# lijrjyan/SDVAR

Measured on AMD Instinct MI355X. Metric: images/s (+ mean accepted tokens/step), VAR-d16 256^2 B=8, d12 draft + d16 verify, per GPU, higher is better.
Workload: dtype f32 (GEMM operands split into 2 fp16 planes to 2^-22, 3 fp16 MFMA products, fp32 accumulate); 1 GPU; BASELINE.json P1: VAR-d16 256^2 B=8/GPU, d12 draft + d16 verify, gamma=2, cfg=1.5 top_k=900 top_p=0.96, acceptance=natural, incl. VQVAE decode (overlapped with the next batch on a 2nd stream); verifier one round behind the draft once gamma = 1; parallelism=1 independent batch shards

## Files before the change

### sdvar_amd/csrc/conv.hip

```cpp
#include <stdlib.h>

#include "common.h"
#include "gemm_plan.h"

#ifdef SDVAR_TIMING_EXPERIMENTS
#define SDVAR_CDBG(a, bit) ((a).dbg & (bit))
#else
#define SDVAR_CDBG(a, bit) 0
#endif

namespace sdvar {


typedef __bf16 bf16x8 __attribute__((ext_vector_type(8)));
typedef _Float16 f16x8 __attribute__((ext_vector_type(8)));
typedef __attribute__((address_space(3))) void* lds_ptr_t;
typedef const __attribute__((address_space(1))) void* glb_ptr_t;

enum { CEPI_BIAS = 0, CEPI_BIAS_RES = 1, CEPI_PARTIAL = 2 };
constexpr int CBM = 256, CBN = 160;
constexpr int CSTAGE = 3 * (CBM + CBN) * 32;
constexpr int CSTAGE_H = 2 * (CBM + CBN) * 32;

struct ConvArgs {
    const uint16_t* X; const uint16_t* W;
    size_t xps, wps;
    size_t x_rows;
    int x_row0;
    const float* wsi;
    const float* bias; const float* res; float* out;
    int M, N, cb, taps, ih, iw, ldo, split, k_per_split;
    double* gn_part; int cpg;
    int up_phase;
    size_t w_phase_stride;
    int dbg;
};

__device__ __forceinline__ void conv_gn_store(const ConvArgs& a, const float* red, const float* piv, int n0, int tm, int phase, int tid) {
    const int col0 = tid * a.cpg;
    if (col0 < CBN && n0 + col0 < a.N) {
        const double n = 256.0, in = 1.0 / 256.0;
        double s = 0.0, m = 0.0;
        for (int c = col0; c < col0 + a.cpg; ++c) {
            double s1 = 0.0, s2 = 0.0;
            for (int w = 0; w < 8; ++w) { s1 += (double)red[w * 160 + c]; s2 += (double)red[1280 + w * 160 + c]; }
            const double sc = n * (double)piv[c] + s1;
            s += sc; m += s2 + (sc * sc - s1 * s1) * in;
        }
        double* o = a.gn_part + ((size_t)(a.up_phase >= 0 ? 4 * tm + phase : tm) * 32 + (n0 + col0) / a.cpg) * 2;
        o[0] = s; o[1] = m - s * s / (n * a.cpg);
    }
}

template <int EPI>
__device__ __forceinline__ void conv_epilogue(const ConvArgs& a, f32x16 (&acc)[5], float wsi, int m0, int n0, int tm, int ks, int phase, int wave, int li, int lh,
                                              int tid, uint16_t* csm) {
    float rv[5][16];
    if (EPI == CEPI_BIAS_RES) {
#pragma unroll
        for (int j = 0; j < 5; ++j) {
            const int n = n0 + j * 32 + li;
#pragma unroll
            for (int r = 0; r < 16; ++r) {
                const int m = m0 + wave * 32 + (r & 3) + 8 * (r >> 2) + 4 * lh;
                rv[j][r] = (n < a.N && m < a.M) ? a.res[(size_t)m * a.ldo + n] : 0.f;
            }
        }
    }
#pragma unroll
// ... 23 lines not shown
        if (wave == 0 && lh == 0) {
#pragma unroll
            for (int j = 0; j < 5; ++j) piv[j * 32 + li] = acc[j][0];
        }
        __syncthreads();
#pragma unroll
        for (int j = 0; j < 5; ++j) {
            float s1 = 0.f, s2 = 0.f;
            if (n0 + j * 32 + li < a.N) {
                const float K = piv[j * 32 + li];
#pragma unroll
                for (int r = 0; r < 16; ++r) { const float d = acc[j][r] - K; s1 += d; s2 += d * d; }
            }
            const auto w1 = __builtin_amdgcn_permlane32_swap(__float_as_uint(s1), __float_as_uint(s1), false, false);
            const auto w2 = __builtin_amdgcn_permlane32_swap(__float_as_uint(s2), __float_as_uint(s2), false, false);
            if (lh == 0) {
                red[wave * 160 + j * 32 + li] = __uint_as_float(w1[0]) + __uint_as_float(w1[1]);
                red[1280 + wave * 160 + j * 32 + li] = __uint_as_float(w2[0]) + __uint_as_float(w2[1]);
            }
        }
        __syncthreads();
        conv_gn_store(a, red, piv, n0, tm, phase, tid);
    }
}

typedef float cf32x4 __attribute__((ext_vector_type(4)));
__device__ __forceinline__ float dpp_row_sum16(float v) {
    v += __builtin_bit_cast(float, __builtin_amdgcn_update_dpp(0, __builtin_bit_cast(int, v), 0x111, 0xF, 0xF, true));
    v += __builtin_bit_cast(float, __builtin_amdgcn_update_dpp(0, __builtin_bit_cast(int, v), 0x112, 0xF, 0xF, true));
    v += __builtin_bit_cast(float, __builtin_amdgcn_update_dpp(0, __builtin_bit_cast(int, v), 0x114, 0xF, 0xF, true));
    v += __builtin_bit_cast(float, __builtin_amdgcn_update_dpp(0, __builtin_bit_cast(int, v), 0x118, 0xF, 0xF, true));
    return v;
}
template <int EPI>
__device__ __forceinline__ void conv_epilogue16(const ConvArgs& a, cf32x4 (&acc)[2][10], float wsi, int m0, int n0, int tm, int ks, int phase, int wave, int l15, int lq,
                                                int tid, uint16_t* csm) {
    int mrow[2]; size_t orow[2];
#pragma unroll
    for (int mt = 0; mt < 2; ++mt) {
        const int m = m0 + wave * 32 + 16 * mt + l15;
        mrow[mt] = m; orow[mt] = (size_t)m;
        if (EPI != CEPI_PARTIAL && a.up_phase >= 0 && m < a.M) {
            const int hw = a.ih * a.iw, b = m / hw, rem = m - b * hw, y = rem / a.iw, x = rem - y * a.iw;
            orow[mt] = ((size_t)(b * 2 * a.ih + 2 * y + (phase >> 1)) * (2 * a.iw) + 2 * x + (phase & 1));
        }
    }
    cf32x4 rv[2][10];
    if (EPI == CEPI_BIAS_RES) {
#pragma unroll
        for (int mt = 0; mt < 2; ++mt)
#pragma unroll
            for (int nt = 0; nt < 10; ++nt) {
                const int n = n0 + 16 * nt + 4 * lq;
                rv[mt][nt] = (n < a.N && mrow[mt] < a.M) ? *reinterpret_cast<const cf32x4*>(a.res + (size_t)mrow[mt] * a.ldo + n) : cf32x4{0.f, 0.f, 0.f, 0.f};
            }
    }
    float* outp = (EPI == CEPI_PARTIAL) ? a.out + (size_t)ks * a.M * a.ldo : a.out;
#pragma unroll
    for (int nt = 0; nt < 10; ++nt) {
        const int n = n0 + 16 * nt + 4 * lq;
        if (n >= a.N) continue;
        const cf32x4 bv = (EPI != CEPI_PARTIAL && a.bias) ? *reinterpret_cast<const cf32x4*>(a.bias + n) : cf32x4{0.f, 0.f, 0.f, 0.f};
#pragma unroll
        for (int mt = 0; mt < 2; ++mt) {
            if (mrow[mt] >= a.M) continue;
            cf32x4 v;
#pragma unroll
            for (int e = 0; e < 4; ++e) { v[e] = acc[mt][nt][e] * wsi + bv[e]; if (EPI == CEPI_BIAS_RES) v[e] += rv[mt][nt][e]; }
            if (!SDVAR_CDBG(a, 4)) *reinterpret_cast<cf32x4*>(outp + orow[mt] * a.ldo + n) = v;
            acc[mt][nt] = v;
        }
    }
    if (EPI != CEPI_PARTIAL && a.gn_part && !SDVAR_CDBG(a, 2)) {
        float* red = reinterpret_cast<float*>(csm);
        __shared__ __attribute__((aligned(16))) float piv[CBN];
        if (wave == 0 && l15 == 0) {
#pragma unroll
            for (int nt = 0; nt < 10; ++nt) *reinterpret_cast<cf32x4*>(piv + 16 * nt + 4 * lq) = acc[0][nt];
        }
        __syncthreads();
#pragma unroll
        for (int nt = 0; nt < 10; ++nt) {
            const bool in = n0 + 16 * nt + 4 * lq < a.N;
            const cf32x4 K = *reinterpret_cast<const cf32x4*>(piv + 16 * nt + 4 * lq);
#pragma unroll
            for (int e = 0; e < 4; ++e) {
                const float x0 = in ? acc[0][nt][e] - K[e] : 0.f, x1 = in ? acc[1][nt][e] - K[e] : 0.f;
                const float s1 = dpp_row_sum16(x0 + x1), s2 = dpp_row_sum16(x0 * x0 + x1 * x1);
                if (l15 == 15) { red[wave * 160 + 16 * nt + 4 * lq + e] = s1; red[1280 + wave * 160 + 16 * nt + 4 * lq + e] = s2; }
            }
        }
        __syncthreads();
        conv_gn_store(a, red, piv, n0, tm, phase, tid);
    }
}

template <int EPI>
__global__ __launch_bounds__(512, 2) void conv_bf16x3_kernel(ConvArgs a) {
    extern __shared__ __attribute__((aligned(16))) uint16_t csm[];
    const int tiles_m = (a.M + CBM - 1) / CBM, tiles_n = (a.N + CBN - 1) / CBN, ntile = tiles_m * tiles_n;
    const int ks = blockIdx.x / ntile;
    const int lid = xcd_remap(blockIdx.x - ks * ntile, ntile);
    const int tm = lid / tiles_n, tn = lid - tm * tiles_n;
// ... 88 lines not shown
                __builtin_amdgcn_sched_barrier(0);
                if (s == 0 && j == 0) {
                    SDVAR_LDS_RD(fb[1][1][4], ab1, 18432);
                    SDVAR_RD_B(1, ab1, 0, 0);
                }
                if (pf) {
                    const int grp = 5 * s + j;
                    issue_one(nst, grp);
                    if (grp >= 8) issue_one(nst, grp + 2);
                }
                __builtin_amdgcn_sched_barrier(0);
            }
        }
#undef SDVAR_RD_B
#undef SDVAR_LDS_RD
    }

    conv_epilogue<EPI>(a, acc, 1.0f, m0, n0, tm, ks, phase, wave, li, lh, tid, csm);
}

template <int EPI, int PP>
__global__ __launch_bounds__(512, 2) void conv_f16x2_kernel(ConvArgs a) {
    extern __shared__ __attribute__((aligned(16))) uint16_t csm[];
    const int tiles_m = (a.M + CBM - 1) / CBM, tiles_n = (a.N + CBN - 1) / CBN, ntile = tiles_m * tiles_n;
    const int ks = blockIdx.x / ntile;
    const int lid = xcd_remap(blockIdx.x - ks * ntile, ntile);
    const int tm = lid / tiles_n, tn = lid - tm * tiles_n;
    const int m0 = tm * CBM, n0 = tn * CBN;

    const int tid = threadIdx.x, lane = tid & 63, wave = tid >> 6;
    const int li = lane & 31, lh = lane >> 5;
    const int phase = a.up_phase >= 0 ? (int)blockIdx.y : 0;
    const uint16_t* Wp = a.W + (size_t)phase * a.w_phase_stride;

    const int r16 = lane >> 2;
    const int xr0 = 32 * wave + r16, xr1 = xr0 + 16, wr0 = 16 * wave + r16, wr1 = 128 + wr0;
    const int cx0 = (lane & 3) ^ ((xr0 >> 2) & 3), cx1 = (lane & 3) ^ ((xr1 >> 2) & 3), cw0 = (lane & 3) ^ ((wr0 >> 2) & 3), cw1 = (lane & 3) ^ ((wr1 >> 2) & 3);
    const int nkt = a.taps * a.cb;
    const int kt0 = ks * a.k_per_split;
    const int nk = min(nkt - kt0, a.k_per_split);
    const int w2 = a.iw + 2;
    auto prow = [&](int m) {
        const int hw = a.ih * a.iw, b = m / hw, rem = m - b * hw, y = rem / a.iw, x = rem - y * a.iw;
        return (size_t)(b * (a.ih + 2) + y + 1) * w2 + x + 1;
    };
    const int swave = __builtin_amdgcn_readfirstlane(wave);
    const uint32_t lx0 = (uint32_t)((a.x_row0 + prow(min(m0 + xr0, a.M - 1))) * 32 + 8 * cx0) * 2u;
    const uint32_t lx1 = (uint32_t)((a.x_row0 + prow(min(m0 + xr1, a.M - 1))) * 32 + 8 * cx1) * 2u;
    const uint32_t lw0 = (uint32_t)(min(n0 + wr0, a.N - 1) * 32 + 8 * cw0) * 2u, lw1 = (uint32_t)(min(n0 + wr1, a.N - 1) * 32 + 8 * cw1) * 2u;
    const bool two_w = swave < 2;
    const char* ux = nullptr; const char* uw = nullptr;
    const int tw = (a.taps == 9) ? 3 : 2;
    int sc = kt0 % a.cb, stap = kt0 / a.cb, sty = stap / tw, stx = stap - sty * tw, skb = kt0;
    auto set_next = [&]() {
        const int shift = (a.taps == 9) ? (sty - 1) * w2 + (stx - 1) : (a.taps == 4) ? (sty - 1 + (phase >> 1)) * w2 + (stx - 1 + (phase & 1)) : 0;
        ux = reinterpret_cast<const char*>(a.X) + ((long long)sc * (long long)a.x_rows + shift) * 64;
        uw = reinterpret_cast<const char*>(Wp) + (size_t)skb * a.N * 64;
        ++skb;
        if (++sc == a.cb) { sc = 0; if (++stx == tw) { stx = 0; ++sty; } }
    };
    auto issue_one = [&](uint16_t* st, int q) {
        if (q < 6) {
            const int p = q / 3, kind = q % 3;
            if (kind == 0) SDVAR_DMA16(lx0, ux + p * a.xps * 2, SDVAR_LDS_ADDR(st + p * 8192 + swave * 1024));
            else if (kind == 1) SDVAR_DMA16(lx1, ux + p * a.xps * 2, SDVAR_LDS_ADDR(st + p * 8192 + swave * 1024 + 512));
            else SDVAR_DMA16(lw0, uw + p * a.wps * 2, SDVAR_LDS_ADDR(st + 2 * 8192 + p * 5120 + swave * 512));
// ... 16 lines not shown
    set_next();
#pragma unroll
    for (int q = 0; q < 8; ++q) issue_one(csm, q);
    if (nk > 1) {
        set_next();
#pragma unroll
        for (int q = 0; q < 8; ++q) issue_one(csm + CSTAGE_H, q);
    }
    if constexpr (PP == 2) {
        const int late = __builtin_amdgcn_readfirstlane(wave >> 2);
        const int l15 = lane & 15, lq = lane >> 4;
        auto wait_next = [&](int t) {
            if (t + 2 < nk) { if (two_w) asm volatile("s_waitcnt vmcnt(8)" ::: "memory"); else asm volatile("s_waitcnt vmcnt(6)" ::: "memory"); }
            else asm volatile("s_waitcnt vmcnt(0)" ::: "memory");
        };
#define SDVAR_C_SLOT() do { __builtin_amdgcn_sched_barrier(0); __builtin_amdgcn_s_barrier(); __builtin_amdgcn_sched_barrier(0); } while (0)
#define SDVAR_LDS_RD(dst, addr, off) asm volatile("ds_read_b128 %0, %1 offset:" #off : "=v"(dst) : "v"(addr) : "memory")
#define SDVAR_C_MFMA16(J0)                                                                                      \
        _Pragma("unroll") for (int j = 0; j < 5; ++j)                                                           \
            _Pragma("unroll") for (int i = 0; i < 2; ++i) {                                                     \
                acc16[i][(J0) + j] = __builtin_amdgcn_mfma_f32_16x16x32_f16(fw[j][0], fx[i][1], acc16[i][(J0) + j], 0, 0, 0);   \
                acc16[i][(J0) + j] = __builtin_amdgcn_mfma_f32_16x16x32_f16(fw[j][1], fx[i][0], acc16[i][(J0) + j], 0, 0, 0);   \
                acc16[i][(J0) + j] = __builtin_amdgcn_mfma_f32_16x16x32_f16(fw[j][0], fx[i][0], acc16[i][(J0) + j], 0, 0, 0);   \
            }
        cf32x4 acc16[2][10];
#pragma unroll
        for (int i = 0; i < 2; ++i)
#pragma unroll
            for (int j = 0; j < 10; ++j)
#pragma unroll
                for (int r = 0; r < 4; ++r) acc16[i][j][r] = 0.f;
        const uint32_t fro = (uint32_t)(l15 * 64 + 16 * (lq ^ ((l15 >> 2) & 3)));
        const uint32_t fxo = (uint32_t)(wave * 32 * 64) + fro, fwo = 32768u + fro;
        wait_next(-1);
        SDVAR_C_SLOT();
        if (late) SDVAR_C_SLOT();
        f16x8 fx[2][2], fw[5][2];
#pragma unroll 1
        for (int t = 0; t < nk; ++t) {
            const bool pf = t + 2 < nk;
            uint16_t* nst = csm + ((t + 2) % 3) * CSTAGE_H;
            const uint32_t sb = (uint32_t)(uintptr_t)(lds_ptr_t)(csm + (t % 3) * CSTAGE_H);
            const uint32_t xa = sb + fxo, wa = sb + fwo;
            SDVAR_LDS_RD(fx[0][0], xa, 0); SDVAR_LDS_RD(fx[0][1], xa, 16384); SDVAR_LDS_RD(fx[1][0], xa, 1024); SDVAR_LDS_RD(fx[1][1], xa, 17408);
            SDVAR_LDS_RD(fw[0][0], wa, 0);    SDVAR_LDS_RD(fw[0][1], wa, 10240); SDVAR_LDS_RD(fw[1][0], wa, 1024); SDVAR_LDS_RD(fw[1][1], wa, 11264);
            SDVAR_LDS_RD(fw[2][0], wa, 2048); SDVAR_LDS_RD(fw[2][1], wa, 12288); SDVAR_LDS_RD(fw[3][0], wa, 3072); SDVAR_LDS_RD(fw[3][1], wa, 13312);
            SDVAR_LDS_RD(fw[4][0], wa, 4096); SDVAR_LDS_RD(fw[4][1], wa, 14336);
            if (pf) {
                set_next();
#pragma unroll
                for (int q = 0; q < 4; ++q) issue_one(nst, q);
            }
            asm volatile("s_waitcnt lgkmcnt(0)" ::: "memory");
            SDVAR_C_SLOT();
            SDVAR_C_MFMA16(0);
            SDVAR_C_SLOT();
            SDVAR_LDS_RD(fw[0][0], wa, 5120); SDVAR_LDS_RD(fw[0][1], wa, 15360); SDVAR_LDS_RD(fw[1][0], wa, 6144); SDVAR_LDS_RD(fw[1][1], wa, 16384);
            SDVAR_LDS_RD(fw[2][0], wa, 7168); SDVAR_LDS_RD(fw[2][1], wa, 17408); SDVAR_LDS_RD(fw[3][0], wa, 8192); SDVAR_LDS_RD(fw[3][1], wa, 18432);
            SDVAR_LDS_RD(fw[4][0], wa, 9216); SDVAR_LDS_RD(fw[4][1], wa, 19456);
            if (pf) {
#pragma unroll
                for (int q = 4; q < 8; ++q) issue_one(nst, q);
            }
            if (late) wait_next(t);
            asm volatile("s_waitcnt lgkmcnt(0)" ::: "memory");
            SDVAR_C_SLOT();
            SDVAR_C_MFMA16(5);
            if (!late) wait_next(t);
            SDVAR_C_SLOT();
        }
        if (!late) SDVAR_C_SLOT();
#undef SDVAR_C_MFMA16
#undef SDVAR_LDS_RD
#undef SDVAR_C_SLOT
        if (SDVAR_CDBG(a, 1)) return;
        conv_epilogue16<EPI>(a, acc16, a.wsi ? *a.wsi : 1.0f, m0, n0, tm, ks, phase, wave, l15, lq, tid, csm);
        return;
    } else
    if (PP) {
        const int late = __builtin_amdgcn_readfirstlane(wave >> 2);
        auto wait_next = [&](int t) {
            if (t + 2 < nk) { if (two_w) asm volatile("s_waitcnt vmcnt(8)" ::: "memory"); else asm volatile("s_waitcnt vmcnt(6)" ::: "memory"); }
            else asm volatile("s_waitcnt vmcnt(0)" ::: "memory");
        };
#define SDVAR_C_SLOT() do { __builtin_amdgcn_sched_barrier(0); __builtin_amdgcn_s_barrier(); __builtin_amdgcn_sched_barrier(0); } while (0)
#define SDVAR_LDS_RD(dst, addr, off) asm volatile("ds_read_b128 %0, %1 offset:" #off : "=v"(dst) : "v"(addr) : "memory")
#define SDVAR_RD_B(ab, p, pb) SDVAR_LDS_RD(fb[p][0], ab, pb); SDVAR_LDS_RD(fb[p][1], ab, pb + 2048); SDVAR_LDS_RD(fb[p][2], ab, pb + 4096); \
                              SDVAR_LDS_RD(fb[p][3], ab, pb + 6144); SDVAR_LDS_RD(fb[p][4], ab, pb + 8192)
#define SDVAR_C_MFMA()                                                                                  \
        _Pragma("unroll") for (int j = 0; j < 5; ++j) {                                                 \
            acc[j] = __builtin_amdgcn_mfma_f32_32x32x16_f16(fa[1], fb[0][j], acc[j], 0, 0, 0);          \
            acc[j] = __builtin_amdgcn_mfma_f32_32x32x16_f16(fa[0], fb[1][j], acc[j], 0, 0, 0);          \
            acc[j] = __builtin_amdgcn_mfma_f32_32x32x16_f16(fa[0], fb[0][j], acc[j], 0, 0, 0);          \
        }
        wait_next(-1);
        SDVAR_C_SLOT();
        if (late) SDVAR_C_SLOT();
        f16x8 fa[2], fb[2][5];
#pragma unroll 1
        for (int t = 0; t < nk; ++t) {
            const bool pf = t + 2 < nk;
            uint16_t* nst = csm + ((t + 2) % 3) * CSTAGE_H;
            const uint32_t sb = (uint32_t)(uintptr_t)(lds_ptr_t)(csm + (t % 3) * CSTAGE_H);
            const uint32_t aa0 = sb + 2 * (offa + ch0), aa1 = sb + 2 * (offa + ch1), ab0 = sb + 2 * (offb + ch0), ab1 = sb + 2 * (offb + ch1);
            SDVAR_LDS_RD(fa[0], aa0, 0); SDVAR_LDS_RD(fa[1], aa0, 16384);
            SDVAR_RD_B(ab0, 0, 0); SDVAR_RD_B(ab0, 1, 10240);
            if (pf) {
                set_next();
#pragma unroll
// ... 34 lines not shown
        f16x8 fa[2][2], fb[2][2][5];
#define SDVAR_LDS_RD(dst, addr, off) asm volatile("ds_read_b128 %0, %1 offset:" #off : "=v"(dst) : "v"(addr) : "memory")
#define SDVAR_RD_B(s, ab, p, pb) SDVAR_LDS_RD(fb[s][p][0], ab, pb); SDVAR_LDS_RD(fb[s][p][1], ab, pb + 2048); SDVAR_LDS_RD(fb[s][p][2], ab, pb + 4096); \
                                 SDVAR_LDS_RD(fb[s][p][3], ab, pb + 6144); SDVAR_LDS_RD(fb[s][p][4], ab, pb + 8192)
        SDVAR_LDS_RD(fa[0][0], aa0, 0); SDVAR_LDS_RD(fa[0][1], aa0, 16384);
        SDVAR_RD_B(0, ab0, 0, 0); SDVAR_RD_B(0, ab0, 1, 10240);
        SDVAR_LDS_RD(fa[1][0], aa1, 0); SDVAR_LDS_RD(fa[1][1], aa1, 16384);
        SDVAR_RD_B(1, ab1, 0, 0); SDVAR_RD_B(1, ab1, 1, 10240);
#undef SDVAR_RD_B
#undef SDVAR_LDS_RD
#pragma unroll
        for (int s = 0; s < 2; ++s) {
            if (s == 0) asm volatile("s_waitcnt lgkmcnt(12)" ::: "memory");
            else asm volatile("s_waitcnt lgkmcnt(0)" ::: "memory");
            __builtin_amdgcn_sched_barrier(0);
#pragma unroll
            for (int j = 0; j < 5; ++j) {
                acc[j] = __builtin_amdgcn_mfma_f32_32x32x16_f16(fa[s][1], fb[s][0][j], acc[j], 0, 0, 0);
                acc[j] = __builtin_amdgcn_mfma_f32_32x32x16_f16(fa[s][0], fb[s][1][j], acc[j], 0, 0, 0);
                acc[j] = __builtin_amdgcn_mfma_f32_32x32x16_f16(fa[s][0], fb[s][0][j], acc[j], 0, 0, 0);
                __builtin_amdgcn_sched_barrier(0);
                if (pf) {
                    const int grp = 5 * s + j;
                    if (grp < 8) issue_one(nst, grp);
                }
                __builtin_amdgcn_sched_barrier(0);
            }
        }
    }
    if (SDVAR_CDBG(a, 1)) return;
    conv_epilogue<EPI>(a, acc, a.wsi ? *a.wsi : 1.0f, m0, n0, tm, ks, phase, wave, li, lh, tid, csm);
}

__global__ __launch_bounds__(256) void conv_reduce_kernel(const float* __restrict__ ws, int split, const float* __restrict__ bias, const float* res,
                                                          float* out, int M, int N) {
    const int nv = N >> 2;
    const size_t total = (size_t)M * nv, slab = (size_t)M * N;
    for (size_t i = (size_t)blockIdx.x * blockDim.x + threadIdx.x; i < total; i += (size_t)gridDim.x * blockDim.x) {
        const int n = (int)(i % nv) * 4;
        f32x4 acc = *reinterpret_cast<const f32x4*>(ws + 4 * i);
        for (int s = 1; s < split; ++s) {
            const f32x4 p = *reinterpret_cast<const f32x4*>(ws + s * slab + 4 * i);
            acc[0] += p[0]; acc[1] += p[1]; acc[2] += p[2]; acc[3] += p[3];
        }
        if (bias) { const f32x4 b = *reinterpret_cast<const f32x4*>(bias + n); acc[0] += b[0]; acc[1] += b[1]; acc[2] += b[2]; acc[3] += b[3]; }
        if (res) { const f32x4 r = *reinterpret_cast<const f32x4*>(res + 4 * i); acc[0] += r[0]; acc[1] += r[1]; acc[2] += r[2]; acc[3] += r[3]; }
        *reinterpret_cast<f32x4*>(out + 4 * i) = acc;
    }
}

__global__ __launch_bounds__(256) void conv_weight_planes_kernel(const float* __restrict__ w, uint16_t* __restrict__ p, int Cout, int Cin, int taps, size_t ps, int pfmt,
                                                                 const float* scale) {
    const int K = taps * Cin;
    const size_t total = (size_t)Cout * K;
    const float sc = (pfmt == PLANES_F16X2 && scale) ? *scale : 1.0f;
    for (size_t i = (size_t)blockIdx.x * blockDim.x + threadIdx.x; i < total; i += (size_t)gridDim.x * blockDim.x) {
        const int co = (int)(i / K), k = (int)(i % K), tap = k / Cin, ci = k - tap * Cin;
        const float v = w[((size_t)co * Cin + ci) * taps + tap];
        const size_t o = kb_index(co, k, Cout);
        if (pfmt == PLANES_F16X2) {
            uint16_t h, l;
            split2h(v * sc, h, l);
            p[o] = h; p[ps + o] = l;
        } else {
            uint16_t p0, p1, p2;
            split3(v, p0, p1, p2);
// ... 34 lines not shown
static int conv_choose_split(int M, int N, int nkt, size_t ws_floats, double kstep_cycles) {
    const long tiles = (long)((M + CBM - 1) / CBM) * ((N + CBN - 1) / CBN);
    double best = 1e30; int bs = 1;
    for (int split = 1; split <= 16 && split <= nkt / 2; ++split) {
        if (split > 1 && ((size_t)split * M * N > ws_floats || N % 4)) break;
        const int kps = (nkt + split - 1) / split;
        if ((nkt + kps - 1) / kps != split) continue;
        const long rounds = (tiles * split + 255) / 256;
        double cyc = (double)rounds * (kps * kstep_cycles + 3000.0);
        if (split > 1) cyc += 4000.0 + (double)(split + 2) * M * N * 4.0 / 4000.0;
        if (cyc < best) { best = cyc; bs = split; }
    }
    return bs;
}

int conv_planes(const uint16_t* X, size_t xps, size_t x_rows, int x_row0, const uint16_t* W, size_t wps, int pfmt, const float* wsi, const float* bias, const float* res,
                float* out, int B, int H, int Wd, int N, int Cin, int taps, float* ws, size_t ws_floats, int force_split, double* gn_part, int* gn_done, int up_phase,
                size_t w_phase_stride, hipStream_t stream) {
    if (gn_done) *gn_done = 0;
    const int M = B * H * Wd, w2 = Wd + 2;
    const size_t Mp = (size_t)B * (H + 2) * w2;
    SDVAR_CHECK_ARG(X && W && out, "conv: null operand");
    SDVAR_CHECK_ARG(M > 0 && N > 0 && Cin > 0 && Cin % 32 == 0 && (taps == 1 || taps == 9 || (taps == 4 && up_phase >= 0)) && (taps == 4 || up_phase < 0), "conv: M=%d N=%d Cin=%d taps=%d", M, N, Cin, taps);
    SDVAR_CHECK_ARG(B > 0 && H > 0 && Wd > 0 && x_row0 >= w2 + 1, "conv: guard rows %d < row pitch %d + 1", x_row0, w2);
    SDVAR_CHECK_ARG(up_phase < 0 || !res, "conv: no residual with the fused up-sampling");
    SDVAR_CHECK_ARG(x_rows >= (size_t)x_row0 + Mp + w2 + 1, "conv: plane rows %zu too few", x_rows);
    SDVAR_CHECK_ARG(((uintptr_t)X % 16) == 0 && ((uintptr_t)W % 16) == 0 && xps % 8 == 0 && wps % 8 == 0, "conv: planes must be 16-byte aligned");
    SDVAR_CHECK_ARG(pfmt == PLANES_BF16X3 || pfmt == PLANES_F16X2, "conv: plane format %d", pfmt);
    const bool F16 = pfmt == PLANES_F16X2;
    ConvArgs a{X, W, xps, wps, x_rows, x_row0, F16 ? wsi : nullptr, bias, res, out, M, N, Cin / 32, taps, H, Wd, N, 1, taps * (Cin / 32), nullptr, 1, up_phase, w_phase_stride, 0};
#ifdef SDVAR_TIMING_EXPERIMENTS
    static const int conv_dbg = getenv("SDVAR_CONV_DBG") ? atoi(getenv("SDVAR_CONV_DBG")) : 0;
    a.dbg = conv_dbg;
#else
    a.dbg = 0;
#endif
    const int nkt = taps * (Cin / 32);
    const int tiles = ((M + CBM - 1) / CBM) * ((N + CBN - 1) / CBN);
    int split = up_phase >= 0 ? 1 : force_split > 0 ? force_split : conv_choose_split(M, N, nkt, ws ? ws_floats : 0, F16 ? 1200.0 : 2100.0);
    if (split > nkt) split = nkt;
    if (split > 1) {
        SDVAR_CHECK_ARG(ws && (size_t)split * M * N <= ws_floats && N % 4 == 0, "conv: split-K workspace too small");
        const int kps = (nkt + split - 1) / split;
        split = (nkt + kps - 1) / kps;
        a.k_per_split = kps; a.split = split;
    }
    const size_t lds = F16 ? 3 * (size_t)CSTAGE_H * sizeof(uint16_t) : 2 * (size_t)CSTAGE * sizeof(uint16_t);
    const int pp_env = variant(VAR_CONV_PP);
    const int pp = (pp_env == 2 && N % 4 != 0) ? 1 : pp_env;
    static LdsOptIn opt_in, opt_in_h;
    if (F16) SDVAR_LDS_OPT_IN(opt_in_h, lds, (const void*)conv_f16x2_kernel<CEPI_BIAS, 0>, (const void*)conv_f16x2_kernel<CEPI_BIAS_RES, 0>, (const void*)conv_f16x2_kernel<CEPI_PARTIAL, 0>,
                              (const void*)conv_f16x2_kernel<CEPI_BIAS, 1>, (const void*)conv_f16x2_kernel<CEPI_BIAS_RES, 1>, (const void*)conv_f16x2_kernel<CEPI_PARTIAL, 1>,
                              (const void*)conv_f16x2_kernel<CEPI_BIAS, 2>, (const void*)conv_f16x2_kernel<CEPI_BIAS_RES, 2>, (const void*)conv_f16x2_kernel<CEPI_PARTIAL, 2>);
    else SDVAR_LDS_OPT_IN(opt_in, lds, (const void*)conv_bf16x3_kernel<CEPI_BIAS>, (const void*)conv_bf16x3_kernel<CEPI_BIAS_RES>, (const void*)conv_bf16x3_kernel<CEPI_PARTIAL>);
    if (split > 1) {
        ConvArgs p = a;
        p.out = ws;
        if (F16 && pp == 2) hipLaunchKernelGGL((conv_f16x2_kernel<CEPI_PARTIAL, 2>), dim3(tiles * split), dim3(512), lds, stream, p);
        else if (F16 && pp) hipLaunchKernelGGL((conv_f16x2_kernel<CEPI_PARTIAL, 1>), dim3(tiles * split), dim3(512), lds, stream, p);
        else if (F16) hipLaunchKernelGGL((conv_f16x2_kernel<CEPI_PARTIAL, 0>), dim3(tiles * split), dim3(512), lds, stream, p);
        else hipLaunchKernelGGL((conv_bf16x3_kernel<CEPI_PARTIAL>), dim3(tiles * split), dim3(512), lds, stream, p);
        SDVAR_LAUNCH_CHECK();
        const size_t total = (size_t)M * (N / 4);
        const int rgrid = (int)((total + 255) / 256 < 4096 ? (total + 255) / 256 : 4096);
        hipLaunchKernelGGL(conv_reduce_kernel, dim3(rgrid), dim3(256), 0, stream, ws, split, bias, res, out, M, N);
        SDVAR_LAUNCH_CHECK();
        return SDVAR_OK;
    }
    if (gn_part && N % 32 == 0 && CBN % (N / 32) == 0 && (H * Wd) % CBM == 0) { a.gn_part = gn_part; a.cpg = N / 32; if (gn_done) *gn_done = 1; }
    if (F16) {
        if (res && pp == 2) hipLaunchKernelGGL((conv_f16x2_kernel<CEPI_BIAS_RES, 2>), dim3(tiles), dim3(512), lds, stream, a);
        else if (res && pp) hipLaunchKernelGGL((conv_f16x2_kernel<CEPI_BIAS_RES, 1>), dim3(tiles), dim3(512), lds, stream, a);
        else if (res) hipLaunchKernelGGL((conv_f16x2_kernel<CEPI_BIAS_RES, 0>), dim3(tiles), dim3(512), lds, stream, a);
        else if (pp == 2) hipLaunchKernelGGL((conv_f16x2_kernel<CEPI_BIAS, 2>), dim3(tiles, up_phase >= 0 ? 4 : 1), dim3(512), lds, stream, a);
        else if (pp) hipLaunchKernelGGL((conv_f16x2_kernel<CEPI_BIAS, 1>), dim3(tiles, up_phase >= 0 ? 4 : 1), dim3(512), lds, stream, a);
        else hipLaunchKernelGGL((conv_f16x2_kernel<CEPI_BIAS, 0>), dim3(tiles, up_phase >= 0 ? 4 : 1), dim3(512), lds, stream, a);
    } else if (res) hipLaunchKernelGGL((conv_bf16x3_kernel<CEPI_BIAS_RES>), dim3(tiles), dim3(512), lds, stream, a);
    else hipLaunchKernelGGL((conv_bf16x3_kernel<CEPI_BIAS>), dim3(tiles, up_phase >= 0 ? 4 : 1), dim3(512), lds, stream, a);
    SDVAR_LAUNCH_CHECK();
    return SDVAR_OK;
}

}
```

### sdvar_amd/csrc/gemm.hip

```cpp
#include "common.h"
#include "gemm_plan.h"

namespace sdvar {

enum { EPI_BIAS = 0, EPI_BIAS_GELU = 1, EPI_GATED_RES = 2, EPI_PARTIAL = 3 };

constexpr int BK = 32;
constexpr int LDS_STRIDE = BK + 4;

struct GemmArgs {
    const float* X; const float* W; const float* bias; float* out;
    const float* res; const float* gate;
    int M, N, K, ldx, ldo, ldres;
    int rows_per_gate, gate_stride;
    int split, k_per_split;
};

template <int BM, int BN, int WAVES_M, int WAVES_N, int EPI>
__global__ __launch_bounds__(256) void gemm_f32_nt_kernel(GemmArgs a) {
    static_assert(WAVES_M * WAVES_N == 4, "4 waves per workgroup");
    constexpr int WM = BM / WAVES_M, WN = BN / WAVES_N;
    constexpr int TM = WM / 32, TN = WN / 32;
    static_assert(TM >= 1 && TN >= 1, "wave tile too small");
    constexpr int XV = BM / 32, WV = BN / 32;
// ... 107 lines not shown
        for (int s = 1; s < split; ++s) {
            const f32x4 p = *reinterpret_cast<const f32x4*>(ws + s * slab + (size_t)m * N + n);
            acc[0] += p[0]; acc[1] += p[1]; acc[2] += p[2]; acc[3] += p[3];
        }
#pragma unroll
        for (int e = 0; e < 4; ++e) {
            float v = acc[e] + (bias ? bias[n + e] : 0.f);
            if (EPI == EPI_BIAS_GELU) v = gelu_tanh(v);
            if (EPI == EPI_GATED_RES) v = res[(size_t)m * ldres + n + e] + v * gate[(size_t)(m / rows_per_gate) * gate_stride + n + e];
            out[(size_t)m * ldo + n + e] = v;
        }
    }
}

static thread_local float* g_ws = nullptr;
constexpr size_t WS_FLOATS = (size_t)24 << 20;

static thread_local float* g_ws_model = nullptr;
float* set_splitk_workspace(float* p) { float* old = g_ws_model; g_ws_model = p; return old; }
size_t splitk_workspace_floats() { return WS_FLOATS; }

float* splitk_workspace(size_t* floats) {
    if (floats) *floats = WS_FLOATS;
    if (g_ws_model) return g_ws_model;
    if (!g_ws && hipMalloc((void**)&g_ws, WS_FLOATS * sizeof(float)) != hipSuccess) { set_error("split-K workspace allocation failed"); return nullptr; }
    return g_ws;
}

Variant g_variants[VAR_COUNT] = {
    {"gemm_h4_var", "SDVAR_GEMM_H4_VAR", 3, 0, 3, 3, false, false},
    {"gemm_h2_stages", "SDVAR_GEMM_H2_STAGES", 6, 2, 6, 6, false, false},
    {"gemm_small_pp", "SDVAR_GEMM_SMALL_PP", 2, 0, 2, 2, false, false},
    {"attn_pp_sched", "SDVAR_ATTN_PP_SCHED", 1, 0, 3, 1, false, false},
    {"conv_pp", "SDVAR_CONV_PP", 2, 0, 2, 2, true, false},
    {"rowblk", "SDVAR_ROWBLK", 1, 0, 2, 1, false, false},
    {"qkv_fuse", "SDVAR_NO_QKV_FUSE", 1, 0, 1, 1, false, true},
    {"gemm_v2", nullptr, 1, 0, 1, 1, false, false},
    {nullptr, nullptr, 0, 0, 768, 0, false, false},
    {nullptr, nullptr, 0, -64, 64, 0, false, false},
};

template <int BM, int BN, int WAVES_M, int WAVES_N, int EPI>
static int launch_f32_kernel(const GemmArgs& a, int grid, hipStream_t stream) {
    const size_t lds = 2 * (size_t)(BM + BN) * LDS_STRIDE * sizeof(float);
    static LdsOptIn opt_in;
    SDVAR_LDS_OPT_IN(opt_in, lds, (const void*)gemm_f32_nt_kernel<BM, BN, WAVES_M, WAVES_N, EPI>);
    hipLaunchKernelGGL((gemm_f32_nt_kernel<BM, BN, WAVES_M, WAVES_N, EPI>), dim3(grid), dim3(256), lds, stream, a);
    SDVAR_LAUNCH_CHECK();
    return SDVAR_OK;
}

static int launch_reduce(const GemmArgs& a, const float* ws, int split, int epi, hipStream_t stream) {
    return dispatch_epi(epi, [&](auto e) {
        hipLaunchKernelGGL(splitk_reduce_kernel<decltype(e)::value>, dim3(splitk_reduce_grid(a.M, a.N)), dim3(256), 0, stream, ws, split, a.bias, a.out, a.res, a.gate, a.M, a.N, a.ldo, a.ldres,
                           a.rows_per_gate, a.gate_stride);
        SDVAR_LAUNCH_CHECK();
        return SDVAR_OK;
    });
}

template <int BM, int BN, int WAVES_M, int WAVES_N>
static int launch_cfg(const GemmArgs& a, int epi, int split, hipStream_t stream) {
    const int tiles = ((a.M + BM - 1) / BM) * ((a.N + BN - 1) / BN);
    return launch_splitk(a, epi, split, tiles, nullptr,
                         [&](const GemmArgs& x, int grid, auto e) { return launch_f32_kernel<BM, BN, WAVES_M, WAVES_N, decltype(e)::value>(x, grid, stream); },
                         [&](const GemmArgs& x, const float* ws, int sp, int ep) { return launch_reduce(x, ws, sp, ep, stream); });
}
// ... 18 lines not shown
```

### sdvar_amd/csrc/gemm_plan.h

```cpp
#pragma once
#include <limits.h>
#include <stdlib.h>
#include <string.h>

#include <atomic>
#include <type_traits>

#include "common.h"

namespace sdvar {

enum VariantId { VAR_GEMM_H4, VAR_GEMM_H2_STAGES, VAR_GEMM_SMALL_PP, VAR_ATTN_PP_SCHED, VAR_CONV_PP, VAR_ROWBLK, VAR_QKV_FUSE, VAR_GEMM_V2, VAR_FORCE_BM, VAR_FORCE_SPLIT, VAR_COUNT };

struct Variant {
    const char* name;
    const char* env;
    int def, lo, hi, fallback;
    bool env_per_call;
    bool env_switches_off;
    std::atomic<int> set{INT_MIN}, cached{INT_MIN};

    int from_env() const {
        const char* e = env ? getenv(env) : nullptr;
        if (!e) return def;
        if (env_switches_off) return 0;
        const int v = atoi(e);
        return v < lo || v > hi ? fallback : v;
    }
    int get() {
        const int s = set.load(std::memory_order_relaxed);
        if (s != INT_MIN && !env_switches_off) return s;
        int c = env_per_call ? from_env() : cached.load(std::memory_order_relaxed);
        if (c == INT_MIN) { c = from_env(); cached.store(c, std::memory_order_relaxed); }
        return (s == INT_MIN || c == 0) ? c : s;
    }
    void store(int v) { set.store(v, std::memory_order_relaxed); }
    void put(int v) { store(v < 0 ? INT_MIN : v); }
};
extern Variant g_variants[VAR_COUNT];
inline int variant(VariantId id) { return g_variants[id].get(); }
inline int set_variant_by_name(const char* name, int value) {
    for (Variant& v : g_variants) {
        if (!v.name || strcmp(v.name, name)) continue;
        SDVAR_CHECK_ARG(value <= v.hi && (value < 0 || value >= v.lo), "%s %d", name, value);
        v.put(value);
// ... 201 lines not shown
```

Before: 186.0 images/s.

## Add persistent f16x2 conv kernel prefetching next tile during epilogue

Adds a persistent conv kernel, selected when SDVAR_CONV_PP=3, that walks tiles in a grid-stride loop. It issues the first two K-stage DMAs of the next tile before running the current epilogue, so the epilogue's output stores overlap with the next tile's loads. Bias is staged into LDS once per tile, and the epilogue gets a fast path with no bounds checks for full tiles. The default conv_pp stays at 2, so the persistent path is opt-in, while the LDS bias staging and full-tile fast path also apply to the existing pp=2 kernel. Timing stamp instrumentation is added under the timing-experiment build flag.

After: 185.9 images/s. No clear change (-0.0%).

```diff
diff --git a/sdvar_amd/csrc/conv.hip b/sdvar_amd/csrc/conv.hip
--- a/sdvar_amd/csrc/conv.hip
+++ b/sdvar_amd/csrc/conv.hip
@@ -34,7 +34,22 @@
     int up_phase;
     size_t w_phase_stride;
     int dbg;
+#ifdef SDVAR_TIMING_EXPERIMENTS
+    unsigned long long* stamps;
+#endif
 };
+
+#ifdef SDVAR_TIMING_EXPERIMENTS
+unsigned long long* debug_get_gemm_stamps();
+constexpr int CONV_STAMP_CUS = 256;
+__device__ __forceinline__ int conv_stamp_slot(int round, int first, int last) {
+    const int i = round == 0 ? 0 : round == 3 ? 1 : round == 7 ? 2 : -1;
+    return (i < 0 || !(first || last)) ? -1 : 2 * i + (first ? 0 : 1);
+}
+#define SDVAR_CSTAMP(k) do { if (st_slot >= 0) st_t[k] = __builtin_amdgcn_s_memrealtime(); } while (0)
+#else
+#define SDVAR_CSTAMP(k) do { } while (0)
+#endif
 
 __device__ __forceinline__ void conv_gn_store(const ConvArgs& a, const float* red, const float* piv, int n0, int tm, int phase, int tid) {
     const int col0 = tid * a.cpg;
@@ -124,9 +139,15 @@
     v += __builtin_bit_cast(float, __builtin_amdgcn_update_dpp(0, __builtin_bit_cast(int, v), 0x118, 0xF, 0xF, true));
     return v;
 }
+__device__ __forceinline__ void conv_stage_bias(const ConvArgs& a, int n0, int tid, float* bias_lds) {
+    if (tid < CBN / 4) {
+        const int n = n0 + 4 * tid;
+        *reinterpret_cast<cf32x4*>(bias_lds + 4 * tid) = (a.bias && n < a.N) ? *reinterpret_cast<const cf32x4*>(a.bias + n) : cf32x4{0.f, 0.f, 0.f, 0.f};
+    }
+}
 template <int EPI>
 __device__ __forceinline__ void conv_epilogue16(const ConvArgs& a, cf32x4 (&acc)[2][10], float wsi, int m0, int n0, int tm, int ks, int phase, int wave, int l15, int lq,
-                                                int tid, uint16_t* csm) {
+                                                int tid, uint16_t* csm, const float* bias_lds) {
     int mrow[2]; size_t orow[2];
 #pragma unroll
     for (int mt = 0; mt < 2; ++mt) {
@@ -137,30 +158,53 @@
             orow[mt] = ((size_t)(b * 2 * a.ih + 2 * y + (phase >> 1)) * (2 * a.iw) + 2 * x + (phase & 1));
         }
     }
-    cf32x4 rv[2][10];
-    if (EPI == CEPI_BIAS_RES) {
-#pragma unroll
-        for (int mt = 0; mt < 2; ++mt)
-#pragma unroll
-            for (int nt = 0; nt < 10; ++nt) {
-                const int n = n0 + 16 * nt + 4 * lq;
-                rv[mt][nt] = (n < a.N && mrow[mt] < a.M) ? *reinterpret_cast<const cf32x4*>(a.res + (size_t)mrow[mt] * a.ldo + n) : cf32x4{0.f, 0.f, 0.f, 0.f};
-            }
-    }
     float* outp = (EPI == CEPI_PARTIAL) ? a.out + (size_t)ks * a.M * a.ldo : a.out;
-#pragma unroll
-    for (int nt = 0; nt < 10; ++nt) {
-        const int n = n0 + 16 * nt + 4 * lq;
-        if (n >= a.N) continue;
-        const cf32x4 bv = (EPI != CEPI_PARTIAL && a.bias) ? *reinterpret_cast<const cf32x4*>(a.bias + n) : cf32x4{0.f, 0.f, 0.f, 0.f};
-#pragma unroll
-        for (int mt = 0; mt < 2; ++mt) {
-            if (mrow[mt] >= a.M) continue;
-            cf32x4 v;
-#pragma unroll
-            for (int e = 0; e < 4; ++e) { v[e] = acc[mt][nt][e] * wsi + bv[e]; if (EPI == CEPI_BIAS_RES) v[e] += rv[mt][nt][e]; }
-            if (!SDVAR_CDBG(a, 4)) *reinterpret_cast<cf32x4*>(outp + orow[mt] * a.ldo + n) = v;
-            acc[mt][nt] = v;
+    if (m0 + CBM <= a.M && n0 + CBN <= a.N) {
+        cf32x4 rv[2][10];
+        if (EPI == CEPI_BIAS_RES) {
+#pragma unroll
+            for (int mt = 0; mt < 2; ++mt)
+#pragma unroll
+                for (int nt = 0; nt < 10; ++nt) rv[mt][nt] = *reinterpret_cast<const cf32x4*>(a.res + (size_t)mrow[mt] * a.ldo + n0 + 16 * nt + 4 * lq);
+        }
+#pragma unroll
+        for (int nt = 0; nt < 10; ++nt) {
+            const int n = n0 + 16 * nt + 4 * lq;
+            const cf32x4 bv = (EPI != CEPI_PARTIAL) ? *reinterpret_cast<const cf32x4*>(bias_lds + 16 * nt + 4 * lq) : cf32x4{0.f, 0.f, 0.f, 0.f};
+#pragma unroll
+            for (int mt = 0; mt < 2; ++mt) {
+                cf32x4 v;
+#pragma unroll
+                for (int e = 0; e < 4; ++e) { v[e] = acc[mt][nt][e] * wsi + bv[e]; if (EPI == CEPI_BIAS_RES) v[e] += rv[mt][nt][e]; }
+                if (!SDVAR_CDBG(a, 4)) *reinterpret_cast<cf32x4*>(outp + orow[mt] * a.ldo + n) = v;
+                acc[mt][nt] = v;
+            }
+        }
+    } else {
+        cf32x4 rv[2][10];
+        if (EPI == CEPI_BIAS_RES) {
+#pragma unroll
+            for (int mt = 0; mt < 2; ++mt)
+#pragma unroll
+                for (int nt = 0; nt < 10; ++nt) {
+                    const int n = n0 + 16 * nt + 4 * lq;
+                    rv[mt][nt] = (n < a.N && mrow[mt] < a.M) ? *reinterpret_cast<const cf32x4*>(a.res + (size_t)mrow[mt] * a.ldo + n) : cf32x4{0.f, 0.f, 0.f, 0.f};
+                }
+        }
+#pragma unroll
+        for (int nt = 0; nt < 10; ++nt) {
+            const int n = n0 + 16 * nt + 4 * lq;
+            if (n >= a.N) continue;
+            const cf32x4 bv = (EPI != CEPI_PARTIAL) ? *reinterpret_cast<const cf32x4*>(bias_lds + 16 * nt + 4 * lq) : cf32x4{0.f, 0.f, 0.f, 0.f};
+#pragma unroll
+            for (int mt = 0; mt < 2; ++mt) {
+                if (mrow[mt] >= a.M) continue;
+                cf32x4 v;
+#pragma unroll
+                for (int e = 0; e < 4; ++e) { v[e] = acc[mt][nt][e] * wsi + bv[e]; if (EPI == CEPI_BIAS_RES) v[e] += rv[mt][nt][e]; }
+                if (!SDVAR_CDBG(a, 4)) *reinterpret_cast<cf32x4*>(outp + orow[mt] * a.ldo + n) = v;
+                acc[mt][nt] = v;
+            }
         }
     }
     if (EPI != CEPI_PARTIAL && a.gn_part && !SDVAR_CDBG(a, 2)) {
@@ -315,6 +359,13 @@
     const int li = lane & 31, lh = lane >> 5;
     const int phase = a.up_phase >= 0 ? (int)blockIdx.y : 0;
     const uint16_t* Wp = a.W + (size_t)phase * a.w_phase_stride;
+#ifdef SDVAR_TIMING_EXPERIMENTS
+    unsigned long long st_t[5] = {0, 0, 0, 0, 0};
+    const int st_w = (int)blockIdx.x % CONV_STAMP_CUS;
+    const int st_slot = (PP == 2 && a.stamps && blockIdx.y == 0 && __builtin_amdgcn_readfirstlane(wave) == 0)
+                            ? conv_stamp_slot((int)blockIdx.x / CONV_STAMP_CUS, st_w == 0, st_w == CONV_STAMP_CUS - 1 || blockIdx.x == gridDim.x - 1) : -1;
+    SDVAR_CSTAMP(0);
+#endif
 
     const int r16 = lane >> 2;
     const int xr0 = 32 * wave + r16, xr1 = xr0 + 16, wr0 = 16 * wave + r16, wr1 = 128 + wr0;
@@ -397,9 +448,12 @@
                 for (int r = 0; r < 4; ++r) acc16[i][j][r] = 0.f;
         const uint32_t fro = (uint32_t)(l15 * 64 + 16 * (lq ^ ((l15 >> 2) & 3)));
         const uint32_t fxo = (uint32_t)(wave * 32 * 64) + fro, fwo = 32768u + fro;
+        __shared__ __attribute__((aligned(16))) float bias_s[CBN];
+        if (EPI != CEPI_PARTIAL) conv_stage_bias(a, n0, tid, bias_s);
         wait_next(-1);
         SDVAR_C_SLOT();
         if (late) SDVAR_C_SLOT();
+        SDVAR_CSTAMP(1);
         f16x8 fx[2][2], fw[5][2];
 #pragma unroll 1
         for (int t = 0; t < nk; ++t) {
@@ -438,8 +492,17 @@
 #undef SDVAR_C_MFMA16
 #undef SDVAR_LDS_RD
 #undef SDVAR_C_SLOT
+        SDVAR_CSTAMP(2);
         if (SDVAR_CDBG(a, 1)) return;
-        conv_epilogue16<EPI>(a, acc16, a.wsi ? *a.wsi : 1.0f, m0, n0, tm, ks, phase, wave, l15, lq, tid, csm);
+        conv_epilogue16<EPI>(a, acc16, a.wsi ? *a.wsi : 1.0f, m0, n0, tm, ks, phase, wave, l15, lq, tid, csm, bias_s);
+#ifdef SDVAR_TIMING_EXPERIMENTS
+        SDVAR_CSTAMP(3);
+        if (st_slot >= 0) {
+            asm volatile("s_waitcnt vmcnt(0)" ::: "memory");
+            SDVAR_CSTAMP(4);
+            if (lane == 0) for (int k = 0; k < 5; ++k) a.stamps[8 * st_slot + k] = st_t[k];
+        }
+#endif
         return;
     } else
     if (PP) {
@@ -540,6 +603,187 @@
     conv_epilogue<EPI>(a, acc, a.wsi ? *a.wsi : 1.0f, m0, n0, tm, ks, phase, wave, li, lh, tid, csm);
 }
 
+template <int EPI>
+__global__ __launch_bounds__(512, 2) void conv_f16x2_persist_kernel(ConvArgs a, int nitem) {
+    extern __shared__ __attribute__((aligned(16))) uint16_t csm[];
+    const int tiles_m = (a.M + CBM - 1) / CBM, tiles_n = (a.N + CBN - 1) / CBN, ntile = tiles_m * tiles_n;
+    const int tid = threadIdx.x, lane = tid & 63, wave = tid >> 6;
+    const int l15 = lane & 15, lq = lane >> 4;
+    const int swave = __builtin_amdgcn_readfirstlane(wave);
+    const int late = swave >> 2;
+    const bool two_w = swave < 2;
+
+    const int r16 = lane >> 2;
+    const int xr0 = 32 * wave + r16, xr1 = xr0 + 16, wr0 = 16 * wave + r16, wr1 = 128 + wr0;
+    const int cx0 = (lane & 3) ^ ((xr0 >> 2) & 3), cx1 = (lane & 3) ^ ((xr1 >> 2) & 3), cw0 = (lane & 3) ^ ((wr0 >> 2) & 3), cw1 = (lane & 3) ^ ((wr1 >> 2) & 3);
+    const int nk = a.taps * a.cb;
+    const int w2 = a.iw + 2;
+    const int tw = (a.taps == 9) ? 3 : 2;
+    auto prow = [&](int m) {
+        const int hw = a.ih * a.iw, b = m / hw, rem = m - b * hw, y = rem / a.iw, x = rem - y * a.iw;
+        return (size_t)(b * (a.ih + 2) + y + 1) * w2 + x + 1;
+    };
+    int dm0 = 0, dn0 = 0, dtm = 0, dphase = 0;
+    uint32_t lx0 = 0, lx1 = 0, lw0 = 0, lw1 = 0;
+    const uint16_t* Wp = a.W;
+    const char* ux = nullptr; const char* uw = nullptr;
+    int sc = 0, sty = 0, stx = 0, skb = 0;
+    auto set_item = [&](int item) {
+        dphase = __builtin_amdgcn_readfirstlane(item / ntile);
+        const int lid = xcd_remap(item - dphase * ntile, ntile);
+        dtm = __builtin_amdgcn_readfirstlane(lid / tiles_n);
+        dm0 = dtm * CBM; dn0 = (lid - dtm * tiles_n) * CBN;
+        Wp = a.W + (size_t)dphase * a.w_phase_stride;
+        lx0 = (uint32_t)((a.x_row0 + prow(min(dm0 + xr0, a.M - 1))) * 32 + 8 * cx0) * 2u;
+        lx1 = (uint32_t)((a.x_row0 + prow(min(dm0 + xr1, a.M - 1))) * 32 + 8 * cx1) * 2u;
+        lw0 = (uint32_t)(min(dn0 + wr0, a.N - 1) * 32 + 8 * cw0) * 2u; lw1 = (uint32_t)(min(dn0 + wr1, a.N - 1) * 32 + 8 * cw1) * 2u;
+        sc = 0; sty = 0; stx = 0; skb = 0;
+    };
+    auto set_next = [&]() {
+        int shift = (a.taps == 9) ? (sty - 1) * w2 + (stx - 1) : (a.taps == 4) ? (sty - 1 + (dphase >> 1)) * w2 + (stx - 1 + (dphase & 1)) : 0;
+        shift = __builtin_amdgcn_readfirstlane(shift);
+        ux = reinterpret_cast<const char*>(a.X) + ((long long)sc * (long long)a.x_rows + shift) * 64;
+        uw = reinterpret_cast<const char*>(Wp) + (size_t)skb * a.N * 64;
+        ++skb;
+        if (++sc == a.cb) { sc = 0; if (++stx == tw) { stx = 0; ++sty; } }
+    };
+    auto issue_one = [&](uint16_t* st, int q) {
+        if (q < 6) {
+            const int p = q / 3, kind = q % 3;
+            if (kind == 0) SDVAR_DMA16(lx0, ux + p * a.xps * 2, SDVAR_LDS_ADDR(st + p * 8192 + swave * 1024));
+            else if (kind == 1) SDVAR_DMA16(lx1, ux + p * a.xps * 2, SDVAR_LDS_ADDR(st + p * 8192 + swave * 1024 + 512));
+            else SDVAR_DMA16(lw0, uw + p * a.wps * 2, SDVAR_LDS_ADDR(st + 2 * 8192 + p * 5120 + swave * 512));
+        } else if (two_w) {
+            const int p = q - 6;
+            SDVAR_DMA16(lw1, uw + p * a.wps * 2, SDVAR_LDS_ADDR(st + 2 * 8192 + p * 5120 + 4096 + swave * 512));
+        }
+    };
+    auto issue_first_two = [&](int item) {
+        set_item(item);
+        set_next();
+#pragma unroll
+        for (int q = 0; q < 8; ++q) issue_one(csm + CSTAGE_H, q);
+        if (nk > 1) {
+            set_next();
+#pragma unroll
+            for (int q = 0; q < 8; ++q) issue_one(csm + 2 * CSTAGE_H, q);
+        }
+    };
+#define SDVAR_C_VMCNT(n) asm volatile("s_waitcnt vmcnt(" #n ")" ::: "memory")
+    auto wait_dma = [&](bool newer, int credit) {
+        if (credit) {
+            if (!newer) SDVAR_C_VMCNT(20);
+            else if (two_w) SDVAR_C_VMCNT(28);
+            else SDVAR_C_VMCNT(26);
+        } else {
+            if (!newer) SDVAR_C_VMCNT(0);
+            else if (two_w) SDVAR_C_VMCNT(8);
+            else SDVAR_C_VMCNT(6);
+        }
+    };
+#define SDVAR_C_SLOT() do { __builtin_amdgcn_sched_barrier(0); __builtin_amdgcn_s_barrier(); __builtin_amdgcn_sched_barrier(0); } while (0)
+#define SDVAR_LDS_RD(dst, addr, off) asm volatile("ds_read_b128 %0, %1 offset:" #off : "=v"(dst) : "v"(addr) : "memory")
+#define SDVAR_C_MFMA16(J0)                                                                                      \
+    _Pragma("unroll") for (int j = 0; j < 5; ++j)                                                               \
+        _Pragma("unroll") for (int i = 0; i < 2; ++i) {                                                         \
+            acc16[i][(J0) + j] = __builtin_amdgcn_mfma_f32_16x16x32_f16(fw[j][0], fx[i][1], acc16[i][(J0) + j], 0, 0, 0);   \
+            acc16[i][(J0) + j] = __builtin_amdgcn_mfma_f32_16x16x32_f16(fw[j][1], fx[i][0], acc16[i][(J0) + j], 0, 0, 0);   \
+            acc16[i][(J0) + j] = __builtin_amdgcn_mfma_f32_16x16x32_f16(fw[j][0], fx[i][0], acc16[i][(J0) + j], 0, 0, 0);   \
+        }
+    const uint32_t fro = (uint32_t)(l15 * 64 + 16 * (lq ^ ((l15 >> 2) & 3)));
+    const uint32_t fxo = (uint32_t)(wave * 32 * 64) + fro, fwo = 32768u + fro;
+    const float wsi = a.wsi ? *a.wsi : 1.0f;
+#ifdef SDVAR_TIMING_EXPERIMENTS
+    unsigned long long st_t[5] = {0, 0, 0, 0, 0};
+    int st_round = 0;
+#endif
+
+    __shared__ __attribute__((aligned(16))) float bias_s[2][CBN];
+    int bias_n0 = -1, bsel = 0;
+
+    int item = blockIdx.x, credit = 0;
+    issue_first_two(item);
+    while (true) {
+        const int m0 = dm0, n0 = dn0, tm = dtm, phase = dphase;
+        if (n0 != bias_n0) {
+            bsel ^= 1;
+            conv_stage_bias(a, n0, tid, bias_s[bsel]);
+            bias_n0 = n0;
+        }
+#ifdef SDVAR_TIMING_EXPERIMENTS
+        const int st_slot = (a.stamps && swave == 0) ? conv_stamp_slot(st_round, blockIdx.x == 0, blockIdx.x == gridDim.x - 1) : -1;
+        ++st_round;
+        SDVAR_CSTAMP(0);
+#endif
+        cf32x4 acc16[2][10];
+#pragma unroll
+        for (int i = 0; i < 2; ++i)
+#pragma unroll
+            for (int j = 0; j < 10; ++j)
+#pragma unroll
+                for (int r = 0; r < 4; ++r) acc16[i][j][r] = 0.f;
+        wait_dma(nk > 1, credit);
+        SDVAR_C_SLOT();
+        if (late) SDVAR_C_SLOT();
+        SDVAR_CSTAMP(1);
+        f16x8 fx[2][2], fw[5][2];
+#pragma unroll 1
+        for (int t = 0; t < nk; ++t) {
+            const bool pf = t + 2 < nk;
+            const int cr = t == 0 ? credit : 0;
+            uint16_t* nst = csm + (t % 3) * CSTAGE_H;
+            const uint32_t sb = (uint32_t)(uintptr_t)(lds_ptr_t)(csm + ((t + 1) % 3) * CSTAGE_H);
+            const uint32_t xa = sb + fxo, wa = sb + fwo;
+            SDVAR_LDS_RD(fx[0][0], xa, 0); SDVAR_LDS_RD(fx[0][1], xa, 16384); SDVAR_LDS_RD(fx[1][0], xa, 1024); SDVAR_LDS_RD(fx[1][1], xa, 17408);
+            SDVAR_LDS_RD(fw[0][0], wa, 0);    SDVAR_LDS_RD(fw[0][1], wa, 10240); SDVAR_LDS_RD(fw[1][0], wa, 1024); SDVAR_LDS_RD(fw[1][1], wa, 11264);
+            SDVAR_LDS_RD(fw[2][0], wa, 2048); SDVAR_LDS_RD(fw[2][1], wa, 12288); SDVAR_LDS_RD(fw[3][0], wa, 3072); SDVAR_LDS_RD(fw[3][1], wa, 13312);
+            SDVAR_LDS_RD(fw[4][0], wa, 4096); SDVAR_LDS_RD(fw[4][1], wa, 14336);
+            if (pf) {
+                set_next();
+#pragma unroll
+                for (int q = 0; q < 4; ++q) issue_one(nst, q);
+            }
+            asm volatile("s_waitcnt lgkmcnt(0)" ::: "memory");
+            SDVAR_C_SLOT();
+            SDVAR_C_MFMA16(0);
+            SDVAR_C_SLOT();
+            SDVAR_LDS_RD(fw[0][0], wa, 5120); SDVAR_LDS_RD(fw[0][1], wa, 15360); SDVAR_LDS_RD(fw[1][0], wa, 6144); SDVAR_LDS_RD(fw[1][1], wa, 16384);
+            SDVAR_LDS_RD(fw[2][0], wa, 7168); SDVAR_LDS_RD(fw[2][1], wa, 17408); SDVAR_LDS_RD(fw[3][0], wa, 8192); SDVAR_LDS_RD(fw[3][1], wa, 18432);
+            SDVAR_LDS_RD(fw[4][0], wa, 9216); SDVAR_LDS_RD(fw[4][1], wa, 19456);
+            if (pf) {
+#pragma unroll
+                for (int q = 4; q < 8; ++q) issue_one(nst, q);
+            }
+            if (late) wait_dma(pf, cr);
+            asm volatile("s_waitcnt lgkmcnt(0)" ::: "memory");
+            SDVAR_C_SLOT();
+            SDVAR_C_MFMA16(5);
+            if (!late) wait_dma(pf, cr);
+            SDVAR_C_SLOT();
+        }
+        if (!late) SDVAR_C_SLOT();
+        SDVAR_CSTAMP(2);
+        const int nxt = item + (int)gridDim.x;
+        const bool more = nxt < nitem;
+        if (more) issue_first_two(nxt);
+        credit = 0;
+        if (!SDVAR_CDBG(a, 1)) {
+            conv_epilogue16<EPI>(a, acc16, wsi, m0, n0, tm, 0, phase, wave, l15, lq, tid, csm, bias_s[bsel]);
+            if (!SDVAR_CDBG(a, 4) && m0 + CBM <= a.M && n0 + CBN <= a.N) credit = 20;
+        }
+#ifdef SDVAR_TIMING_EXPERIMENTS
+        SDVAR_CSTAMP(3);
+        if (st_slot >= 0 && lane == 0) for (int k = 0; k < 4; ++k) a.stamps[8 * st_slot + k] = st_t[k];
+#endif
+        if (!more) break;
+        item = nxt;
+    }
+#undef SDVAR_C_MFMA16
+#undef SDVAR_LDS_RD
+#undef SDVAR_C_SLOT
+#undef SDVAR_C_VMCNT
+}
+
 __global__ __launch_bounds__(256) void conv_reduce_kernel(const float* __restrict__ ws, int split, const float* __restrict__ bias, const float* res,
                                                           float* out, int M, int N) {
     const int nv = N >> 2;
@@ -640,6 +884,7 @@
 #ifdef SDVAR_TIMING_EXPERIMENTS
     static const int conv_dbg = getenv("SDVAR_CONV_DBG") ? atoi(getenv("SDVAR_CONV_DBG")) : 0;
     a.dbg = conv_dbg;
+    a.stamps = debug_get_gemm_stamps();
 #else
     a.dbg = 0;
 #endif
@@ -655,11 +900,14 @@
     }
     const size_t lds = F16 ? 3 * (size_t)CSTAGE_H * sizeof(uint16_t) : 2 * (size_t)CSTAGE * sizeof(uint16_t);
     const int pp_env = variant(VAR_CONV_PP);
-    const int pp = (pp_env == 2 && N % 4 != 0) ? 1 : pp_env;
+    const bool persist = pp_env == 3 && F16 && split == 1 && N % 4 == 0;
+    const int pp2 = pp_env == 3 ? 2 : pp_env;
+    const int pp = (pp2 == 2 && N % 4 != 0) ? 1 : pp2;
     static LdsOptIn opt_in, opt_in_h;
     if (F16) SDVAR_LDS_OPT_IN(opt_in_h, lds, (const void*)conv_f16x2_kernel<CEPI_BIAS, 0>, (const void*)conv_f16x2_kernel<CEPI_BIAS_RES, 0>, (const void*)conv_f16x2_kernel<CEPI_PARTIAL, 0>,
                               (const void*)conv_f16x2_kernel<CEPI_BIAS, 1>, (const void*)conv_f16x2_kernel<CEPI_BIAS_RES, 1>, (const void*)conv_f16x2_kernel<CEPI_PARTIAL, 1>,
-                              (const void*)conv_f16x2_kernel<CEPI_BIAS, 2>, (const void*)conv_f16x2_kernel<CEPI_BIAS_RES, 2>, (const void*)conv_f16x2_kernel<CEPI_PARTIAL, 2>);
+                              (const void*)conv_f16x2_kernel<CEPI_BIAS, 2>, (const void*)conv_f16x2_kernel<CEPI_BIAS_RES, 2>, (const void*)conv_f16x2_kernel<CEPI_PARTIAL, 2>,
+                              (const void*)conv_f16x2_persist_kernel<CEPI_BIAS>, (const void*)conv_f16x2_persist_kernel<CEPI_BIAS_RES>);
     else SDVAR_LDS_OPT_IN(opt_in, lds, (const void*)conv_bf16x3_kernel<CEPI_BIAS>, (const void*)conv_bf16x3_kernel<CEPI_BIAS_RES>, (const void*)conv_bf16x3_kernel<CEPI_PARTIAL>);
     if (split > 1) {
         ConvArgs p = a;
@@ -676,7 +924,20 @@
         return SDVAR_OK;
     }
     if (gn_part && N % 32 == 0 && CBN % (N / 32) == 0 && (H * Wd) % CBM == 0) { a.gn_part = gn_part; a.cpg = N / 32; if (gn_done) *gn_done = 1; }
-    if (F16) {
+    if (persist) {
+        static std::atomic<int> cus{0};
+        int ncu = cus.load(std::memory_order_relaxed);
+        if (!ncu) {
+            int dev = 0;
+            SDVAR_HIP(hipGetDevice(&dev));
+            SDVAR_HIP(hipDeviceGetAttribute(&ncu, hipDeviceAttributeMultiprocessorCount, dev));
+            cus.store(ncu, std::memory_order_relaxed);
+        }
+        const int nitem = tiles * (up_phase >= 0 ? 4 : 1), cap = variant(VAR_CONV_GRID) > 0 ? variant(VAR_CONV_GRID) : ncu;
+        const int grid = nitem < cap ? nitem : cap;
+        if (res) hipLaunchKernelGGL((conv_f16x2_persist_kernel<CEPI_BIAS_RES>), dim3(grid), dim3(512), lds, stream, a, nitem);
+        else hipLaunchKernelGGL((conv_f16x2_persist_kernel<CEPI_BIAS>), dim3(grid), dim3(512), lds, stream, a, nitem);
+    } else if (F16) {
         if (res && pp == 2) hipLaunchKernelGGL((conv_f16x2_kernel<CEPI_BIAS_RES, 2>), dim3(tiles), dim3(512), lds, stream, a);
         else if (res && pp) hipLaunchKernelGGL((conv_f16x2_kernel<CEPI_BIAS_RES, 1>), dim3(tiles), dim3(512), lds, stream, a);
         else if (res) hipLaunchKernelGGL((conv_f16x2_kernel<CEPI_BIAS_RES, 0>), dim3(tiles), dim3(512), lds, stream, a);
diff --git a/sdvar_amd/csrc/gemm.hip b/sdvar_amd/csrc/gemm.hip
--- a/sdvar_amd/csrc/gemm.hip
+++ b/sdvar_amd/csrc/gemm.hip
@@ -163,7 +163,8 @@
     {"gemm_h2_stages", "SDVAR_GEMM_H2_STAGES", 6, 2, 6, 6, false, false},
     {"gemm_small_pp", "SDVAR_GEMM_SMALL_PP", 2, 0, 2, 2, false, false},
     {"attn_pp_sched", "SDVAR_ATTN_PP_SCHED", 1, 0, 3, 1, false, false},
-    {"conv_pp", "SDVAR_CONV_PP", 2, 0, 2, 2, true, false},
+    {"conv_pp", "SDVAR_CONV_PP", 2, 0, 3, 2, true, false},
+    {"conv_grid", nullptr, 0, 0, 1024, 0, false, false},
     {"rowblk", "SDVAR_ROWBLK", 1, 0, 2, 1, false, false},
     {"qkv_fuse", "SDVAR_NO_QKV_FUSE", 1, 0, 1, 1, false, true},
     {"gemm_v2", nullptr, 1, 0, 1, 1, false, false},
diff --git a/sdvar_amd/csrc/gemm_plan.h b/sdvar_amd/csrc/gemm_plan.h
--- a/sdvar_amd/csrc/gemm_plan.h
+++ b/sdvar_amd/csrc/gemm_plan.h
@@ -10,7 +10,7 @@
 
 namespace sdvar {
 
-enum VariantId { VAR_GEMM_H4, VAR_GEMM_H2_STAGES, VAR_GEMM_SMALL_PP, VAR_ATTN_PP_SCHED, VAR_CONV_PP, VAR_ROWBLK, VAR_QKV_FUSE, VAR_GEMM_V2, VAR_FORCE_BM, VAR_FORCE_SPLIT, VAR_COUNT };
+enum VariantId { VAR_GEMM_H4, VAR_GEMM_H2_STAGES, VAR_GEMM_SMALL_PP, VAR_ATTN_PP_SCHED, VAR_CONV_PP, VAR_CONV_GRID, VAR_ROWBLK, VAR_QKV_FUSE, VAR_GEMM_V2, VAR_FORCE_BM, VAR_FORCE_SPLIT, VAR_COUNT };
 
 struct Variant {
     const char* name;
```
